# norlab-ulaval/mask_bev

Hardware: AMD Instinct MI355X
Metric: LiDAR scans/sec fwd+bwd, 120k-pt 512x512 BEV 100q (higher is better)
Workload: dtype bf16; 1 GPU; semantic_kitti_512: 120000 pts/scan, 512x512 BEV, 100 queries; scans_per_gpu=4, global_batch=4, parallelism=dp1, step=fwd + Hungarian loss + bwd + AdamW; inputs device-resident, launch=hip-graph, tuned_gemm_table=True, k3_adam_fused=True

## Files before the change

include/maskbev_hip.h:

```cpp
#ifndef MASKBEV_HIP_H_
#define MASKBEV_HIP_H_

#include <stddef.h>
#include <stdint.h>

#ifdef __cplusplus
extern "C" {
#endif

typedef enum {
  MBV_OK = 0,
  MBV_ERR_BAD_ARG = -1,
  MBV_ERR_WORKSPACE = -2,
  MBV_ERR_UNSUPPORTED = -3
} mbv_status;

int mbv_abi_version(void);

#define MBV_DT_F32 0
#define MBV_DT_BF16 1
#define MBV_DT_F16 2

size_t mbv_voxelize_workspace_bytes(int64_t total_points, int32_t batch, int64_t cells_per_scan);

// ... 349 lines not shown
                      int64_t stride_w, int64_t stride_acc, void* stream);

size_t mbv_gemm16_nn_workspace_bytes(int64_t m, int64_t k, int32_t batch);

int mbv_gemm16_nn(const void* g, const void* w, void* out, const void* aux, float* colsum, int64_t m, int64_t n,
                  int64_t k, int64_t ldg, int64_t ldw, int64_t ldo, int64_t ldaux, int32_t dtype, int32_t out_f32,
                  int32_t act, int32_t batch, int64_t stride_g, int64_t stride_w, int64_t stride_o, void* workspace,
                  size_t workspace_bytes, void* stream);

int64_t mbv_gemm16_nn_part_rows(int64_t m, int64_t k, int32_t batch);

int mbv_gemm16_nn_parts(const void* g, const void* w, void* out, const void* aux, float* parts, size_t parts_bytes,
                        int64_t m, int64_t n, int64_t k, int64_t ldg, int64_t ldw, int64_t ldo, int64_t ldaux,
                        int32_t dtype, int32_t out_f32, int32_t act, int32_t batch, int64_t stride_g, int64_t stride_w,
                        int64_t stride_o, void* stream);

size_t mbv_gemm16_tn_workspace_bytes(int64_t m, int64_t n, int64_t k);

int mbv_gemm16_tn(const void* g, const void* x, void* dw, int64_t m, int64_t n, int64_t k, int64_t ldg, int64_t ldx,
                  int64_t lddw, int32_t dtype, int32_t accumulate, int32_t out_f32, int32_t splits, int32_t batch,
                  int64_t stride_g, int64_t stride_x, int64_t stride_dw, void* workspace, size_t workspace_bytes,
                  void* stream);

int mbv_upsample_bilinear_bwd(const void* grad_out, int32_t grad_dtype, int64_t planes, int32_t h, int32_t w, int32_t in_h,
                              int32_t in_w, void* grad_in, int32_t in_dtype, void* stream);

int mbv_groupnorm_supported(int32_t channels, int32_t groups, int32_t h, int32_t w);
size_t mbv_groupnorm_workspace_bytes(int64_t batch, int32_t channels, int32_t groups, int32_t h, int32_t w);
int mbv_groupnorm_fwd(const void* x, int32_t x_dtype, int64_t batch, int32_t channels, int32_t h, int32_t w,
                      int32_t groups, const float* gamma, const float* beta, float eps, const void* add,
// ... 228 lines not shown
```

mask_bev_amd/_lib.py:

```python
from __future__ import annotations

import ctypes
import os
from ctypes import c_double, c_float, c_int32, c_int64, c_size_t, c_void_p
from typing import Dict, List, Tuple

_PKG_DIR = os.path.dirname(os.path.abspath(__file__))
LIB_PATH = os.path.join(_PKG_DIR, 'libmaskbev_hip.so')

ABI_VERSION = 59


class MaskBevHipError(RuntimeError):
    pass


_P = c_void_p
_F = c_float
_I = c_int32
_L = c_int64
_D = c_double

SIGNATURES: Dict[str, Tuple[object, List[object]]] = {
    'mbv_abi_version': (ctypes.c_int, []),
# ... 99 lines not shown
    'mbv_mask_logits_fwd': (ctypes.c_int, [_P, _P, _I, _I, _I, _I, _L, _P, _I, _P]),
    'mbv_attn_mask_from_logits': (ctypes.c_int, [_P, _I, _L, _I, _I, _I, _I, _P, _P]),
    'mbv_attn_workspace_bytes': (c_size_t, [_I, _I, _I, _I, _I]),
    'mbv_attn_fwd': (ctypes.c_int, [_P, _P, _P, _P, _I, _I, _I, _I, _I, _I, _P, _P, _P, c_size_t, _P]),
    'mbv_attn_bwd': (ctypes.c_int, [_P, _P, _P, _P, _P, _P, _P, _I, _I, _I, _I, _I, _I, _P, _P, _P, _P]),
    'mbv_attn_fwd_ld': (ctypes.c_int, [_P, _P, _P, _I, _P, _I, _I, _I, _I, _I, _I, _P, _P, _P, c_size_t, _P]),
    'mbv_gemm16_supported': (ctypes.c_int, [_I, _L, _L, _L]),
    'mbv_gemm16_nt': (ctypes.c_int, [_P, _P, _P, _P, _P, _L, _L, _L, _L, _L, _L, _I, _I, _I, _I, _L, _L, _L, _P]),
    'mbv_gemm16_nt_acc': (ctypes.c_int, [_P, _P, _P, _L, _L, _L, _L, _L, _L, _I, _I, _I, _L, _L, _L, _P]),
    'mbv_gemm16_nn_workspace_bytes': (c_size_t, [_L, _L, _I]),
    'mbv_gemm16_nn': (ctypes.c_int, [_P, _P, _P, _P, _P, _L, _L, _L, _L, _L, _L, _L, _I, _I, _I, _I, _L, _L, _L, _P,
                                     c_size_t, _P]),
    'mbv_gemm16_nn_part_rows': (ctypes.c_int64, [_L, _L, _I]),
    'mbv_gemm16_nn_parts': (ctypes.c_int, [_P, _P, _P, _P, _P, c_size_t, _L, _L, _L, _L, _L, _L, _L, _I, _I, _I, _I, _L,
                                           _L, _L, _P]),
    'mbv_gemm16_tn_workspace_bytes': (c_size_t, [_L, _L, _L]),
    'mbv_gemm16_tn': (ctypes.c_int, [_P, _P, _P, _L, _L, _L, _L, _L, _L, _I, _I, _I, _I, _I, _L, _L, _L, _P, c_size_t,
                                     _P]),
    'mbv_attn_bwd_ld': (ctypes.c_int, [_P, _P, _P, _I, _P, _P, _P, _P, _I, _I, _I, _I, _I, _I, _P, _P, _P, _I, _I, _P]),
    'mbv_msda_query_inputs': (ctypes.c_int, [_P, _P, _L, _L, _I, _I, _P, _P, _P]),
    'mbv_upsample_bilinear_bwd': (ctypes.c_int, [_P, _I, _L, _I, _I, _I, _I, _P, _I, _P]),
    'mbv_groupnorm_supported': (ctypes.c_int, [_I, _I, _I, _I]),
    'mbv_groupnorm_workspace_bytes': (c_size_t, [_L, _I, _I, _I, _I]),
    'mbv_groupnorm_fwd': (ctypes.c_int, [_P, _I, _L, _I, _I, _I, _I, _P, _P, _F, _P, _I, _I, _I, _I, _P, _I, _P, _P, _P,
                                         c_size_t, _P]),
    'mbv_groupnorm_bwd': (ctypes.c_int, [_P, _I, _P, _I, _P, _P, _P, _P, _L, _I, _I, _I, _I, _I, _P, _I, _P, _P, _I, _P,
                                         _P]),
    'mbv_gemm16_tn_group_workspace_bytes': (c_size_t, [_P, _P, _P, _I]),
    'mbv_gemm32s_supported': (ctypes.c_int, [_I, _L, _L, _L]),
    'mbv_f32_absmax_group': (ctypes.c_int, [_P, _P, _P, _P, _P, _I, _P]),
# ... 126 lines not shown
```

mask_bev_amd/csrc/gemm.hip:

```cpp

#include "common.hpp"
#include "gemm_tiles.hpp"

namespace {

template <int KB, int NS, int WM = 2, int TM = 2, int TN = 2>
struct Geo {
  static constexpr int NW = 2 * WM;
  static constexpr int BM = 32 * TM * WM, BN = 64 * TN;
  static constexpr int SA = (BM + 127) / 128, SB = (BN + 127) / 128;
  static constexpr int IMG = 128 * KB * 2;
  static constexpr int STAGE = (SA + SB) * IMG;
  static constexpr int PPS = IMG / 1024;
  static constexpr int PIECES = (SA + SB) * PPS;
  static constexpr int NP = (PIECES + NW - 1) / NW;
  static constexpr int STG = NW * 32 * STG_LD * 4;
  static constexpr int LDS = NS * STAGE > STG ? NS * STAGE : STG;
  static constexpr int BLOCKS = LDS <= 40960 ? 4 : (LDS <= 53248 ? 3 : (LDS <= 81920 ? 2 : 1));
  static constexpr int WPS = (BLOCKS * NW + 3) / 4 > 8 ? 8 : (BLOCKS * NW + 3) / 4;
};

enum { EPI_NONE = 0, EPI_RELU = 1, EPI_GELU = 2, EPI_DRELU = 3, EPI_DGELU = 4,
       EPI_CONV = 5 };

// ... 3 lines not shown
  void* c;
  void* c2;
  const void* aux;
  const float* bias;
  float* colsum_rows;
  int gm, gn, gk;
  int lda, ldb, ldc, ldx;
  long long sa, sb, sc;
  long long ssplit;
  unsigned a_bytes, b_bytes;
  int ntm, ntn, splits, ksteps;
  int out_f32;
  int acc_out;
  int tap_steps;
  int tap[9];
};

template <int KB, int NS, int WM, int TM, int TN, bool A_KS, bool B_KS, int OUT, int EPI, typename T>
__device__ __forceinline__ void gemm16_body(const GemmArgs& p, const int bid, char* smem) {
  using G = Geo<KB, NS, WM, TM, TN>;
  static_assert(OUT == 1 || TN == 2, "the STORE epilogue turns 64-column wave tiles");
  constexpr int BM = G::BM, BN = G::BN;
  const int tid = threadIdx.x, lane = tid & 63;
  const int wave = __builtin_amdgcn_readfirstlane(tid >> 6);
  const int wm = wave >> 1, wn = wave & 1;

  const int tiles = p.ntm * p.ntn;
  const int z = bid / tiles, t = bid - z * tiles;
  const int tile_m = t / p.ntn, tile_n = t - tile_m * p.ntn;
  const int bz = z / p.splits, sp = z - bz * p.splits;
// ... 205 lines not shown
      s += __shfl_xor(s, 32, 64);
      csum[e] = s;
    }
    if (prow == 0 && col_ok) {
      float* d = p.colsum_rows + ((size_t)bz * WM * p.ntm + WM * tile_m + wm) * (size_t)p.gn + gn;
      *reinterpret_cast<float4*>(d) = make_float4(csum[0], csum[1], csum[2], csum[3]);
      *reinterpret_cast<float4*>(d + 4) = make_float4(csum[4], csum[5], csum[6], csum[7]);
    }
  }
}

template <int KB, int NS, int WM, int TM, int TN, bool A_KS, bool B_KS, int OUT, int EPI, typename T>
__global__ void __launch_bounds__(64 * 2 * WM, (Geo<KB, NS, WM, TM, TN>::WPS)) k_gemm16(const GemmArgs p) {
  extern __shared__ __attribute__((aligned(16))) char smem[];
  gemm16_body<KB, NS, WM, TM, TN, A_KS, B_KS, OUT, EPI, T>(p, xcd_contiguous(blockIdx.x, gridDim.x), smem);
}

constexpr int kTnGroup = 48;
struct TnEntry {
  const void* g; const void* x; float* out;
  int m, n, k, ldg, ldx, ldo;
  int ntn, splits, ksteps, item_begin;
};
struct TnGroupArgs {
  TnEntry e[kTnGroup];
  int n, total_items;
};

template <int KB, int NS, typename T>
__global__ void __launch_bounds__(256, (Geo<KB, NS, 2, 2, 2>::WPS)) k_gemm16_tn_group(const TnGroupArgs a) {
// ... 177 lines not shown
  int s = splits;
  if (s <= 0) {
    const long long tiles = (long long)a.ntm * a.ntn * batch;
    constexpr int target = 512;
    s = (int)((target + tiles - 1) / tiles);
    if (s > total_steps * KB / 256) s = total_steps * KB / 256;
  }
  if (s < 1) s = 1;
  if (s > total_steps) s = total_steps;
  a.ksteps = (total_steps + s - 1) / s;
  a.splits = (total_steps + a.ksteps - 1) / a.ksteps;
}

static bool fits_2g(long long rows, long long ld) { return rows * ld * 2 < 0x7fff0000LL; }

extern "C" int mbv_gemm16_supported(int32_t layout, int64_t m, int64_t n, int64_t k) {
  if (layout < 0 || layout > 2 || m <= 0 || n <= 0 || k <= 0) return 0;
  if ((n & 7) || (k & 7)) return 0;
  return m * (n > k ? n : k) * 2 < 0x7fff0000LL ? 1 : 0;
}

extern "C" int mbv_gemm16_nt(const void* x, const void* w, const float* bias, void* out, void* out_pre, int64_t m,
                             int64_t n, int64_t k, int64_t ldx, int64_t ldw, int64_t ldo, int32_t dtype,
                             int32_t out_f32, int32_t act, int32_t batch, int64_t stride_x, int64_t stride_w,
                             int64_t stride_o, void* stream) {
  if (m < 0 || n <= 0 || k <= 0 || batch < 0 || !x || !w || !out) return MBV_ERR_BAD_ARG;
  if (dtype < 0 || dtype > 1 || act < 0 || act > 2) return MBV_ERR_BAD_ARG;
  if ((n & 7) || (k & 7) || (ldx & 7) || (ldw & 7) || (ldo & 7) || ldx < k || ldw < k || ldo < n) return MBV_ERR_UNSUPPORTED;
  if ((reinterpret_cast<size_t>(x) | reinterpret_cast<size_t>(w) | reinterpret_cast<size_t>(out) |
       reinterpret_cast<size_t>(out_pre) | reinterpret_cast<size_t>(bias)) & 15)
    return MBV_ERR_UNSUPPORTED;
  if (!fits_2g(m, ldx) || !fits_2g(n, ldw)) return MBV_ERR_UNSUPPORTED;
  if (m == 0 || batch == 0) return MBV_OK;
  const int shape = gemm16_pick_shape(0, m, n, batch);
  const int BM = SHAPE_BM[shape], BN = SHAPE_BN[shape];
  GemmArgs a = {};
  a.a = x; a.b = w; a.c = out; a.c2 = out_pre; a.bias = bias;
  a.gm = (int)m; a.gn = (int)n; a.gk = (int)k;
  a.lda = (int)ldx; a.ldb = (int)ldw; a.ldc = (int)ldo;
  a.sa = stride_x; a.sb = stride_w; a.sc = stride_o;
  a.a_bytes = (unsigned)(((m - 1) * ldx + k) * 2); a.b_bytes = (unsigned)(((n - 1) * ldw + k) * 2);
  a.ntm = (int)((m + BM - 1) / BM); a.ntn = (int)((n + BN - 1) / BN); a.splits = 1; a.ksteps = (int)((k + KB - 1) / KB);
  a.out_f32 = out_f32;
  return gemm16_launch(shape, 0, 0, act, dtype, a, batch, (hipStream_t)stream);
}

extern "C" int mbv_gemm16_nt_acc(const void* x, const void* w, float* acc, int64_t m, int64_t n, int64_t k, int64_t ldx,
                                 int64_t ldw, int64_t ldacc, int32_t dtype, int32_t splits, int32_t batch,
                                 int64_t stride_x, int64_t stride_w, int64_t stride_acc, void* stream) {
  if (m < 0 || n <= 0 || k <= 0 || batch < 0 || !x || !w || !acc) return MBV_ERR_BAD_ARG;
  if (dtype < 0 || dtype > 1) return MBV_ERR_BAD_ARG;
  if ((n & 7) || (k & 7) || (ldx & 7) || (ldw & 7) || ldx < k || ldw < k || ldacc < n) return MBV_ERR_UNSUPPORTED;
  if ((reinterpret_cast<size_t>(x) | reinterpret_cast<size_t>(w) | reinterpret_cast<size_t>(acc)) & 15) return MBV_ERR_UNSUPPORTED;
  if (!fits_2g(m, ldx) || !fits_2g(n, ldw)) return MBV_ERR_UNSUPPORTED;
  if (m == 0 || batch == 0) return MBV_OK;
  const int shape = gemm16_pick_shape(1, m, n, (long long)batch * ((k + 511) / 512));
  const int BM = SHAPE_BM[shape], BN = SHAPE_BN[shape];
  GemmArgs a = {};
  a.a = x; a.b = w; a.c = acc;
// ... 35 lines not shown
}

extern "C" size_t mbv_gemm16_nn_workspace_bytes(int64_t m, int64_t k, int32_t batch) {
  return (size_t)((m + 63) / 64 + 4) * (size_t)k * 4 * (size_t)(batch > 0 ? batch : 1);
}

extern "C" int64_t mbv_gemm16_nn_part_rows(int64_t m, int64_t k, int32_t batch) {
  if (m <= 0 || k <= 0 || batch <= 0) return 0;
  const int BM = SHAPE_BM[gemm16_pick_shape(0, m, k, batch)];
  return (int64_t)(BM / 64) * ((m + BM - 1) / BM) * batch;
}

static int gemm16_nn_impl(const void* g, const void* w, void* out, const void* aux, float* colsum, bool parts_only, int64_t m,
                          int64_t n, int64_t k, int64_t ldg, int64_t ldw, int64_t ldo, int64_t ldaux, int32_t dtype,
                          int32_t out_f32, int32_t act, int32_t batch, int64_t stride_g, int64_t stride_w,
                          int64_t stride_o, void* workspace, size_t workspace_bytes, void* stream) {
  if (m < 0 || n <= 0 || k <= 0 || batch < 0 || !g || !w || !out) return MBV_ERR_BAD_ARG;
  if (dtype < 0 || dtype > 1 || act < 0 || act > 2 || (act && !aux)) return MBV_ERR_BAD_ARG;
  if ((n & 7) || (k & 7) || (ldg & 7) || (ldw & 7) || (ldo & 7) || (ldaux & 7) || ldg < n || ldw < k || ldo < k)
    return MBV_ERR_UNSUPPORTED;
  if ((reinterpret_cast<size_t>(g) | reinterpret_cast<size_t>(w) | reinterpret_cast<size_t>(out) |
       reinterpret_cast<size_t>(aux) | reinterpret_cast<size_t>(workspace)) & 15)
    return MBV_ERR_UNSUPPORTED;
  if (!fits_2g(m, ldg) || !fits_2g(n, ldw)) return MBV_ERR_UNSUPPORTED;
  const bool sums = colsum != nullptr || parts_only;
  if (sums && (!workspace || workspace_bytes < mbv_gemm16_nn_workspace_bytes(m, k, batch))) return MBV_ERR_WORKSPACE;
  if (m == 0 || batch == 0) return MBV_OK;
  const int shape = gemm16_pick_shape(0, m, k, batch);
  const int BM = SHAPE_BM[shape], BN = SHAPE_BN[shape];
  GemmArgs a = {};
  a.a = g; a.b = w; a.c = out; a.aux = aux; a.colsum_rows = sums ? reinterpret_cast<float*>(workspace) : nullptr;
  a.gm = (int)m; a.gn = (int)k; a.gk = (int)n;
  a.lda = (int)ldg; a.ldb = (int)ldw; a.ldc = (int)ldo; a.ldx = (int)ldaux;
  a.sa = stride_g; a.sb = stride_w; a.sc = stride_o;
  a.a_bytes = (unsigned)(((m - 1) * ldg + n) * 2); a.b_bytes = (unsigned)(((n - 1) * ldw + k) * 2);
  a.ntm = (int)((m + BM - 1) / BM); a.ntn = (int)((k + BN - 1) / BN); a.splits = 1; a.ksteps = (int)((n + KB - 1) / KB);
  a.out_f32 = out_f32;
  const int rc = gemm16_launch(shape, 1, 0, act == 0 ? EPI_NONE : (act == 1 ? EPI_DRELU : EPI_DGELU), dtype, a, batch,
                               (hipStream_t)stream);
  if (rc != MBV_OK || !colsum || parts_only) return rc;
  const int rows = (BM / 64) * a.ntm * batch;
  int gy = rows / 16;
  if (gy < 1) gy = 1;
  if (gy > 32) gy = 32;
  hipLaunchKernelGGL(k_sum_rows, dim3((unsigned)((k + 63) / 64), (unsigned)gy), dim3(256), 0, (hipStream_t)stream,
                     reinterpret_cast<const float*>(workspace), rows, (int)k, colsum);
  MBV_CHECK_LAUNCH();
  return MBV_OK;
}

extern "C" int mbv_gemm16_nn(const void* g, const void* w, void* out, const void* aux, float* colsum, int64_t m,
                             int64_t n, int64_t k, int64_t ldg, int64_t ldw, int64_t ldo, int64_t ldaux, int32_t dtype,
                             int32_t out_f32, int32_t act, int32_t batch, int64_t stride_g, int64_t stride_w,
                             int64_t stride_o, void* workspace, size_t workspace_bytes, void* stream) {
  return gemm16_nn_impl(g, w, out, aux, colsum, false, m, n, k, ldg, ldw, ldo, ldaux, dtype, out_f32, act, batch, stride_g,
                        stride_w, stride_o, workspace, workspace_bytes, stream);
}

extern "C" int mbv_gemm16_nn_parts(const void* g, const void* w, void* out, const void* aux, float* parts, size_t parts_bytes,
                                   int64_t m, int64_t n, int64_t k, int64_t ldg, int64_t ldw, int64_t ldo, int64_t ldaux,
                                   int32_t dtype, int32_t out_f32, int32_t act, int32_t batch, int64_t stride_g,
                                   int64_t stride_w, int64_t stride_o, void* stream) {
  if (!parts) return MBV_ERR_BAD_ARG;
  return gemm16_nn_impl(g, w, out, aux, nullptr, true, m, n, k, ldg, ldw, ldo, ldaux, dtype, out_f32, act, batch, stride_g,
                        stride_w, stride_o, parts, parts_bytes, stream);
}

extern "C" size_t mbv_gemm16_tn_workspace_bytes(int64_t m, int64_t n, int64_t k) {
  const long long tiles = ((n + 127) / 128) * ((k + 127) / 128);
  long long s = (512 + tiles - 1) / tiles;
  const long long cap = (m + 255) / 256;
  if (s > cap) s = cap;
  if (s < 1) s = 1;
  return (size_t)(s + 1) * (size_t)n * (size_t)k * 4;
}

extern "C" int mbv_gemm16_tn(const void* g, const void* x, void* dw, int64_t m, int64_t n, int64_t k, int64_t ldg,
                             int64_t ldx, int64_t lddw, int32_t dtype, int32_t accumulate, int32_t out_f32,
                             int32_t splits, int32_t batch, int64_t stride_g, int64_t stride_x, int64_t stride_dw,
                             void* workspace, size_t workspace_bytes, void* stream) {
// ... 129 lines not shown
```

mask_bev_amd/ops_gemm_kernels.py:

```python
from __future__ import annotations

import ctypes
from typing import Optional

import torch

from . import _lib, switches
from ._lib import MaskBevHipError, check
from .ops_records import *


_GEMM16_DT = {torch.bfloat16: 0, torch.float16: 1}
_ACT = {None: 0, 'none': 0, 'relu': 1, 'gelu': 2}


def gemm16_enabled() -> bool:
    return switches.get('gemm16') != '0'


def gemm16_policy() -> str:
    v = switches.get('gemm16')
    return {'1': 'auto', '0': 'none'}.get(v, v)


def _k17_min_tokens(kind: str) -> Optional[int]:
    return {'fused': switches.get('k17_fused_min'), 'wgrad': 4096}.get(kind)


def _k17_wants(kind: str, tokens: int) -> bool:
    pol = gemm16_policy()
    if pol == 'none':
        return False
    if pol == 'all':
        return True
    floor = _k17_min_tokens(kind)
    return floor is not None and tokens >= floor


def _gemm16_ok(*ts: torch.Tensor) -> bool:
    dt = ts[0].dtype
    return (dt in _GEMM16_DT and all(t.is_cuda and t.dtype == dt and t.dim() == 2 and t.stride(1) == 1
                                     and t.stride(0) % 8 == 0 and t.shape[1] % 8 == 0 and t.data_ptr() % 16 == 0
                                     and t.shape[0] * t.stride(0) * 2 < 0x7fff0000 for t in ts))


def gemm16_nt(x: torch.Tensor, w: torch.Tensor, bias: Optional[torch.Tensor] = None, act: Optional[str] = None,
              out_dtype: Optional[torch.dtype] = None, want_pre: bool = False):
    lib = _lib.load()
    if not _gemm16_ok(x, w) or x.shape[1] != w.shape[1]:
        raise MaskBevHipError('gemm16_nt: unsupported operands')
    m, k = x.shape
    n = w.shape[0]
    od = out_dtype or x.dtype
    if od not in (x.dtype, torch.float32):
        raise MaskBevHipError('gemm16_nt: out dtype must be the input dtype or f32')
    out = torch.empty((m, n), dtype=od, device=x.device)
    pre = torch.empty((m, n), dtype=od, device=x.device) if (want_pre and _ACT[act]) else None
    if bias is not None and (bias.dtype != torch.float32 or not bias.is_contiguous() or bias.data_ptr() % 16):
        raise MaskBevHipError('gemm16_nt: bias must be contiguous f32, 16-byte aligned')
    check(lib.mbv_gemm16_nt(_ptr(x), _ptr(w), _ptr(bias), _ptr(out), _ptr(pre), m, n, k, x.stride(0), w.stride(0), n,
                            _GEMM16_DT[x.dtype], int(od == torch.float32), _ACT[act], 1, 0, 0, 0, _stream()),
          'mbv_gemm16_nt')
    return (out, pre) if want_pre else out


def gemm16_nn(g: torch.Tensor, w: torch.Tensor, act: Optional[str] = None, aux: Optional[torch.Tensor] = None,
              colsum: Optional[torch.Tensor] = None, out_dtype: Optional[torch.dtype] = None, colsum_sink=None) -> torch.Tensor:
    lib = _lib.load()
    if not _gemm16_ok(g, w) or g.shape[1] != w.shape[0]:
        raise MaskBevHipError('gemm16_nn: unsupported operands')
    m, n = g.shape
    k = w.shape[1]
    a = _ACT[act]
    if a and (aux is None or not _gemm16_ok(aux) or aux.dtype != g.dtype or tuple(aux.shape) != (m, k)):
        raise MaskBevHipError('gemm16_nn: aux must be a (M, K) tensor of the input dtype')
    od = out_dtype or g.dtype
    out = torch.empty((m, k), dtype=od, device=g.device)
    if colsum is not None and (colsum.dtype != torch.float32 or not colsum.is_contiguous()):
        raise MaskBevHipError('gemm16_nn: colsum must be contiguous f32')
    if colsum is not None and colsum_sink is not None:
        rows = int(lib.mbv_gemm16_nn_part_rows(m, k, 1))
        parts = torch.empty(int(lib.mbv_gemm16_nn_workspace_bytes(m, k, 1)) // 4, dtype=torch.float32, device=g.device)
        check(lib.mbv_gemm16_nn_parts(_ptr(g), _ptr(w), _ptr(out), _ptr(aux if a else None), _ptr(parts), parts.numel() * 4,
# ... 225 lines not shown
```

mask_bev_amd/switches.py:

```python
from __future__ import annotations

import contextlib
import os
from typing import Any, Dict

_DEFAULTS: Dict[str, Any] = {
    'decoder_fused': 'auto',
    'deferred_heads': True,
    'shared_kv': True,
    'early_targets': True,
    'wgrad_group': True,
    'tn_group': '1',
    'nn_colsum_defer': True,
    'gemm16': 'auto',
    'tn_max_in': 1536,
    'k17_fused_min': 4096,
    'gemm32s': True,
    'amax_hints': True,
    'amax_verify': False,
    'ffn32': True,
    'k4_split': True,
    'k6_split': True,
    'msda_packed_f32': True,
    'ln_bound_hints': True,
    'conv3x3_k20': True,
    'tn32_group': True,
    'gemm32s_min': 1024,
    'pfn_stream_stats': True,
    'pfn_one_call': True,
# ... 60 lines not shown
```

scratch/pmc_to_json.py:

```python
import collections
import csv
import json
import re
import sys

FAMILIES = [
    ('k_gemm16<TN>', r'k_gemm16I.*Lb1ELb1ELi0E', [r'k_add_parts']),
    ('k_gemm16_tn_group', r'k_gemm16_tn_group', [r'k_add_parts_group']),
    ('k_gn_fwd', r'k_gn_apply', [r'k_gn_stats']),
    ('k_gn_bwd', r'k_gn_bwd_dx', [r'k_gn_bwd_sums']),
    ('k_gemm16<NN>', r'k_gemm16I.*Lb0ELb1ELi0E', [r'k_sum_rows']),
    ('k_gemm16<NT>', r'k_gemm16I.*Lb0ELb0ELi0ELi[0-4]E', []),
    ('k_gemm16<NT,conv3x3>', r'k_gemm16I.*Lb0ELb0ELi0ELi5E', []),
    ('k_gemm32s<NT>', r'k_gemm32sILb0ELb0ELi[012]ELi0E|k_gemm32s<false, false, [012], 0>', []),
    ('k_gemm32s<NT,patch>', r'k_gemm32sILb0ELb0ELi0ELi1E|k_gemm32s<false, false, 0, 1>', []),
    ('k_gemm32s<NT,conv3x3>', r'k_gemm32sILb0ELb0ELi0ELi4E|k_gemm32s<false, false, 0, 4>', []),
    ('k_conv_pad_rows', r'k_(un)?pad_rows', []),
    ('k_gemm32s<NN>', r'k_gemm32sILb0ELb1ELi0ELi0E|k_gemm32s<false, true, 0, 0>', []),
    ('k_gemm32s<NN,dact>', r'k_gemm32sILb0ELb1ELi[34]ELi0E|k_gemm32s<false, true, [34], 0>', []),
    ('k_gemm32s<NN,patch>', r'k_gemm32sILb0ELb1ELi0ELi2E|k_gemm32s<false, true, 0, 2>', []),
    ('k_gemm32s<TN>', r'k_gemm32sILb1ELb1ELi0ELi0E|k_gemm32s<true, true, 0, 0>', [r'k_add_parts32']),
    ('k_gemm32s<TN,patch>', r'k_gemm32sILb1ELb1ELi0ELi3E|k_gemm32s<true, true, 0, 3>', []),
    ('k_gemm32s_tn_group', r'k_gemm32s_tn_group', []),
    ('k_absmax_group', r'k_absmax_group', []),
    ('k_adamw', r'k_adamw', []),
    ('k_sample_select', r'k_sample_select', []),
    ('k_window_attn_bwd', r'k_window_attn(_split)?_bwd', []),
# ... 91 lines not shown
```

Measured before the change: 180.6 scans/s.

## Add LDS-resident A-panel GEMM kernel for small-M activated NT/NN GEMMs

Adds a k_gemm16_panel kernel that loads a 128-row A panel with its full K extent into LDS once. It then sweeps a range of N tiles, streaming B through a multi-stage ring buffer, and fuses the bias, activation and colsum epilogues. The scheduler picks how many N ranges to split each panel into based on the CU count. The path is used by default for activated GEMMs with M≤4096 and K≤256, and aims to avoid reloading A for every output tile and to improve occupancy on small GEMMs. The cost is a large LDS footprint and a new code path that needs careful vmcnt bookkeeping.

Measured after the change: 180.2 scans/s. Within noise of the previous version (-0.2%).

```diff
diff --git a/include/maskbev_hip.h b/include/maskbev_hip.h
--- a/include/maskbev_hip.h
+++ b/include/maskbev_hip.h
@@ -387,6 +387,17 @@
                         int64_t m, int64_t n, int64_t k, int64_t ldg, int64_t ldw, int64_t ldo, int64_t ldaux,
                         int32_t dtype, int32_t out_f32, int32_t act, int32_t batch, int64_t stride_g, int64_t stride_w,
                         int64_t stride_o, void* stream);
+
+int mbv_gemm16_panel_nt(const void* x, const void* w, const float* bias, void* out, void* out_pre, int64_t m, int64_t n,
+                        int64_t k, int64_t ldx, int64_t ldw, int64_t ldo, int32_t dtype, int32_t out_f32, int32_t act,
+                        int32_t batch, int64_t stride_x, int64_t stride_w, int64_t stride_o, int32_t n_ranges, void* stream);
+
+int mbv_gemm16_panel_nn(const void* g, const void* w, void* out, const void* aux, float* colsum, int64_t m, int64_t n,
+                        int64_t k, int64_t ldg, int64_t ldw, int64_t ldo, int64_t ldaux, int32_t dtype, int32_t out_f32,
+                        int32_t act, int32_t batch, int64_t stride_g, int64_t stride_w, int64_t stride_o, void* workspace,
+                        size_t workspace_bytes, int32_t n_ranges, void* stream);
+
+int mbv_gemm16_panel_mode(int32_t mode);
 
 size_t mbv_gemm16_tn_workspace_bytes(int64_t m, int64_t n, int64_t k);
 
diff --git a/mask_bev_amd/_lib.py b/mask_bev_amd/_lib.py
--- a/mask_bev_amd/_lib.py
+++ b/mask_bev_amd/_lib.py
@@ -137,6 +137,10 @@
     'mbv_gemm16_nn_part_rows': (ctypes.c_int64, [_L, _L, _I]),
     'mbv_gemm16_nn_parts': (ctypes.c_int, [_P, _P, _P, _P, _P, c_size_t, _L, _L, _L, _L, _L, _L, _L, _I, _I, _I, _I, _L,
                                            _L, _L, _P]),
+    'mbv_gemm16_panel_nt': (ctypes.c_int, [_P, _P, _P, _P, _P, _L, _L, _L, _L, _L, _L, _I, _I, _I, _I, _L, _L, _L, _I, _P]),
+    'mbv_gemm16_panel_nn': (ctypes.c_int, [_P, _P, _P, _P, _P, _L, _L, _L, _L, _L, _L, _L, _I, _I, _I, _I, _L, _L, _L, _P,
+                                           c_size_t, _I, _P]),
+    'mbv_gemm16_panel_mode': (ctypes.c_int, [_I]),
     'mbv_gemm16_tn_workspace_bytes': (c_size_t, [_L, _L, _L]),
     'mbv_gemm16_tn': (ctypes.c_int, [_P, _P, _P, _L, _L, _L, _L, _L, _L, _I, _I, _I, _I, _I, _L, _L, _L, _P, c_size_t,
                                      _P]),
diff --git a/mask_bev_amd/csrc/gemm.hip b/mask_bev_amd/csrc/gemm.hip
--- a/mask_bev_amd/csrc/gemm.hip
+++ b/mask_bev_amd/csrc/gemm.hip
@@ -1,3 +1,5 @@
+
+#include <atomic>
 
 #include "common.hpp"
 #include "gemm_tiles.hpp"
@@ -41,6 +43,8 @@
   int acc_out;
   int tap_steps;
   int tap[9];
+  int nranges;
+  int part_rows;
 };
 
 template <int KB, int NS, int WM, int TM, int TN, bool A_KS, bool B_KS, int OUT, int EPI, typename T>
@@ -276,6 +280,227 @@
 __global__ void __launch_bounds__(64 * 2 * WM, (Geo<KB, NS, WM, TM, TN>::WPS)) k_gemm16(const GemmArgs p) {
   extern __shared__ __attribute__((aligned(16))) char smem[];
   gemm16_body<KB, NS, WM, TM, TN, A_KS, B_KS, OUT, EPI, T>(p, xcd_contiguous(blockIdx.x, gridDim.x), smem);
+}
+
+template <int N>
+__device__ __forceinline__ void wait_vm() { asm volatile("s_waitcnt vmcnt(%0)" ::"n"(N) : "memory"); }
+
+template <int BASE>
+__device__ __forceinline__ void wait_vm_plus(int e) {
+  switch (e) {
+    case 2: wait_vm<BASE + 2>(); break;
+    case 4: wait_vm<BASE + 4>(); break;
+    case 6: wait_vm<BASE + 6>(); break;
+    case 8: wait_vm<BASE + 8>(); break;
+    case 10: wait_vm<BASE + 10>(); break;
+    case 12: wait_vm<BASE + 12>(); break;
+    case 14: wait_vm<BASE + 14>(); break;
+    default: wait_vm<BASE>(); break;
+  }
+}
+
+template <int KB, int NS>
+struct PanelGeo {
+  static constexpr int NW = 8, BM = 128, BN = 128;
+  static constexpr int IMG = 128 * KB * 2;
+  static_assert(IMG / 1024 == NW, "one LDS-DMA piece per wave and sub-image");
+  static constexpr int RING = NS * IMG;
+  static constexpr int SROWS = 16;
+  static constexpr int STG = NW * SROWS * STG_LD * 4;
+  static constexpr int MAX_K = 384;
+  static constexpr int lds_bytes(int ksteps) { return RING + STG + ksteps * IMG; }
+};
+
+template <int KB, int NS, bool B_KS, int EPI, typename T>
+__global__ void __launch_bounds__(512, 2) k_gemm16_panel(const GemmArgs p) {
+  using G = PanelGeo<KB, NS>;
+  extern __shared__ __attribute__((aligned(16))) char smem[];
+  const int tid = threadIdx.x, lane = tid & 63;
+  const int wave = __builtin_amdgcn_readfirstlane(tid >> 6);
+  const int wm = wave >> 1, wn = wave & 1;
+  const int bid = xcd_contiguous(blockIdx.x, gridDim.x);
+  const int pm = bid / p.nranges, rg = bid - pm * p.nranges;
+  const int t_begin = (int)((long long)rg * p.ntn / p.nranges), t_end = (int)((long long)(rg + 1) * p.ntn / p.nranges);
+  const int nk = p.ksteps, m0 = pm * G::BM;
+
+  char* ring = smem;
+  float* stg = reinterpret_cast<float*>(smem + G::RING) + wave * (G::SROWS * STG_LD);
+  char* panel = smem + G::RING + G::STG;
+  const i32x4 ra = make_rsrc(p.a, p.a_bytes), rb = make_rsrc(p.b, p.b_bytes);
+  const unsigned ring_addr = lds_addr_of(ring), panel_addr = lds_addr_of(panel);
+
+  for (int kt = 0; kt < nk; ++kt)
+    glds16(ra, panel_addr + kt * G::IMG + wave * 1024,
+           piece_offset<KB, false>(0, wave, m0, p.gm, p.lda * 2, kt * KB, p.gk, lane), 0u);
+
+  int st_t = t_begin, st_k = 0, st_slot = 0;
+  auto stage = [&]() {
+    unsigned v = OOB;
+    if (st_t < t_end) v = piece_offset<KB, B_KS>(0, wave, st_t * G::BN, p.gn, p.ldb * 2, st_k * KB, p.gk, lane);
+    glds16(rb, ring_addr + st_slot * G::IMG + wave * 1024, v, 0u);
+    if (++st_k == nk) { st_k = 0; ++st_t; }
+    if (++st_slot == NS) st_slot = 0;
+  };
+#pragma unroll
+  for (int s = 0; s < NS - 1; ++s) stage();
+
+  const int r = lane & 31, h = lane >> 5;
+  const int prow = lane >> 3, cg = lane & 7;
+  const int mrow0 = m0 + 32 * wm + prow;
+  constexpr bool HAS_AUX = EPI == EPI_DRELU || EPI == EPI_DGELU;
+  int slot = 0;
+  const int loads_epi = (HAS_AUX ? 4 : 0) + (p.bias ? 2 : 0);
+  const int stores_full = 4 * (((EPI == EPI_RELU || EPI == EPI_GELU) && p.c2) ? 2 : 1);
+  int younger = loads_epi;
+  for (int t = t_begin; t < t_end; ++t) {
+    const int gn = t * G::BN + 64 * wn + 8 * cg;
+    const bool col_ok = gn < p.gn;
+    const bool full = m0 + 32 * wm + 32 <= p.gm && t * G::BN + 64 * wn + 64 <= p.gn;
+    uint4 auxv[4];
+    if (HAS_AUX) {
+#pragma unroll
+      for (int q = 0; q < 4; ++q) {
+        const int gm = mrow0 + 8 * q;
+        const size_t off = (gm < p.gm && col_ok) ? (size_t)gm * p.ldx + gn : 0;
+        auxv[q] = *reinterpret_cast<const uint4*>(reinterpret_cast<const unsigned short*>(p.aux) + off);
+      }
+    }
+    float bias8[8], csum[8];
+#pragma unroll
+    for (int e = 0; e < 8; ++e) { bias8[e] = 0.f; csum[e] = 0.f; }
+    if (p.bias) {
+      const float* bp = p.bias + (col_ok ? gn : 0);
+      const float4 b0 = *reinterpret_cast<const float4*>(bp);
+      const float4 b1 = *reinterpret_cast<const float4*>(bp + 4);
+      bias8[0] = b0.x; bias8[1] = b0.y; bias8[2] = b0.z; bias8[3] = b0.w;
+      bias8[4] = b1.x; bias8[5] = b1.y; bias8[6] = b1.z; bias8[7] = b1.w;
+    }
+    f32x16 acc[2];
+#pragma unroll
+    for (int j = 0; j < 2; ++j)
+#pragma unroll
+      for (int e = 0; e < 16; ++e) acc[j][e] = 0.f;
+    for (int kt = 0; kt < nk; ++kt) {
+      if (kt <= NS - 2) wait_vm_plus<NS - 2>(younger);
+      else wait_vm<NS - 2>();
+      __syncthreads();
+      stage();
+      const char* aimg = panel + kt * G::IMG;
+      const char* bimg = ring + slot * G::IMG;
+      uint4 af[KB / 16], bf[KB / 16][2];
+#pragma unroll
+      for (int ks = 0; ks < KB / 16; ++ks) {
+        af[ks] = frag_kc<KB>(aimg, 32 * wm, ks, lane);
+#pragma unroll
+        for (int j = 0; j < 2; ++j)
+          bf[ks][j] = B_KS ? frag_ks(bimg, 64 * wn + 32 * j, ks, lane) : frag_kc<KB>(bimg, 64 * wn + 32 * j, ks, lane);
+      }
+#pragma unroll
+      for (int ks = 0; ks < KB / 16; ++ks)
+#pragma unroll
+        for (int j = 0; j < 2; ++j) acc[j] = Mma<T>::run(bf[ks][j], af[ks], acc[j]);
+      if (++slot == NS) slot = 0;
+    }
+
+    younger = loads_epi + (full ? stores_full : 0);
+
+#pragma unroll
+    for (int hf = 0; hf < 2; ++hf) {
+      if (hf) __syncthreads();
+      if ((r >> 4) == hf) {
+#pragma unroll
+        for (int j = 0; j < 2; ++j)
+#pragma unroll
+          for (int g = 0; g < 4; ++g) {
+            f32x4 v;
+            v[0] = acc[j][4 * g]; v[1] = acc[j][4 * g + 1]; v[2] = acc[j][4 * g + 2]; v[3] = acc[j][4 * g + 3];
+            *reinterpret_cast<f32x4*>(stg + (r & 15) * STG_LD + 32 * j + 8 * g + 4 * h) = v;
+          }
+      }
+      __syncthreads();
+      if (hf == 0) {
+#pragma unroll
+        for (int e = 0; e < 8; ++e) asm volatile("" : "+v"(bias8[e]));
+        if (HAS_AUX) {
+#pragma unroll
+          for (int q = 0; q < 4; ++q) asm volatile("" : "+v"(auxv[q].x), "+v"(auxv[q].y), "+v"(auxv[q].z), "+v"(auxv[q].w));
+        }
+      }
+#pragma unroll
+      for (int ps = 0; ps < 2; ++ps) {
+        const int row = 8 * ps + prow, q = 2 * hf + ps;
+        const int gm = mrow0 + 8 * q;
+        const f32x4 lo = *reinterpret_cast<const f32x4*>(stg + row * STG_LD + 8 * cg);
+        const f32x4 hi = *reinterpret_cast<const f32x4*>(stg + row * STG_LD + 8 * cg + 4);
+        if (gm >= p.gm || !col_ok) continue;
+        float v[8] = {lo[0], lo[1], lo[2], lo[3], hi[0], hi[1], hi[2], hi[3]};
+#pragma unroll
+        for (int e = 0; e < 8; ++e) v[e] += bias8[e];
+        const size_t o = (size_t)gm * p.ldc + gn;
+        if (EPI == EPI_RELU || EPI == EPI_GELU) {
+          if (p.c2) store8<T>(p.c2, o, v, p.out_f32);
+          if (!p.out_f32) round8<T>(v);
+#pragma unroll
+          for (int e = 0; e < 8; ++e) {
+            if (EPI == EPI_RELU) {
+              v[e] = v[e] > 0.f ? v[e] : 0.f;
+            } else {
+              float dens;
+              v[e] *= gelu_cdf_parts(v[e], dens);
+            }
+          }
+        } else if (HAS_AUX) {
+          const unsigned w[4] = {auxv[q].x, auxv[q].y, auxv[q].z, auxv[q].w};
+#pragma unroll
+          for (int e = 0; e < 8; ++e) {
+            const float zz = Mma<T>::to_f((unsigned short)(w[e >> 1] >> (16 * (e & 1))));
+            if (EPI == EPI_DRELU) {
+              v[e] = zz > 0.f ? v[e] : 0.f;
+            } else {
+              float dens;
+              const float cdf = gelu_cdf_parts(zz, dens);
+              v[e] *= cdf + zz * dens;
+            }
+          }
+        }
+        store8<T>(p.c, o, v, p.out_f32);
+        if (p.colsum_rows) {
+          if (!p.out_f32) round8<T>(v);
+#pragma unroll
+          for (int e = 0; e < 8; ++e) csum[e] += v[e];
+        }
+      }
+    }
+    if (p.colsum_rows) {
+#pragma unroll
+      for (int e = 0; e < 8; ++e) {
+        float s = csum[e];
+        s += __shfl_xor(s, 8, 64);
+        s += __shfl_xor(s, 16, 64);
+        s += __shfl_xor(s, 32, 64);
+        csum[e] = s;
+      }
+      if ((wm & 1) && prow == 0) {
+        *reinterpret_cast<f32x4*>(stg + 8 * cg) = f32x4{csum[0], csum[1], csum[2], csum[3]};
+        *reinterpret_cast<f32x4*>(stg + 8 * cg + 4) = f32x4{csum[4], csum[5], csum[6], csum[7]};
+      }
+      __syncthreads();
+      if (!(wm & 1) && prow == 0 && col_ok) {
+        const float* o = stg + 2 * (G::SROWS * STG_LD);
+        const f32x4 o0 = *reinterpret_cast<const f32x4*>(o + 8 * cg), o1 = *reinterpret_cast<const f32x4*>(o + 8 * cg + 4);
+        float* d = p.colsum_rows + (size_t)(2 * pm + (wm >> 1)) * (size_t)p.gn + gn;
+        *reinterpret_cast<float4*>(d) = make_float4(csum[0] + o0[0], csum[1] + o0[1], csum[2] + o0[2], csum[3] + o0[3]);
+        *reinterpret_cast<float4*>(d + 4) = make_float4(csum[4] + o1[0], csum[5] + o1[1], csum[6] + o1[2], csum[7] + o1[3]);
+        if (pm == p.ntm - 1)
+          for (int row = 2 * p.ntm + (wm >> 1); row < p.part_rows; row += 2) {
+            float* z = p.colsum_rows + (size_t)row * (size_t)p.gn + gn;
+            *reinterpret_cast<float4*>(z) = make_float4(0.f, 0.f, 0.f, 0.f);
+            *reinterpret_cast<float4*>(z + 4) = make_float4(0.f, 0.f, 0.f, 0.f);
+          }
+      }
+    }
+  }
+  asm volatile("s_waitcnt vmcnt(0)" ::: "memory");
 }
 
 constexpr int kTnGroup = 48;
@@ -483,23 +708,113 @@
 
 static bool fits_2g(long long rows, long long ld) { return rows * ld * 2 < 0x7fff0000LL; }
 
+using PG = PanelGeo<KB, NS>;
+constexpr int NS_DEEP = 6;
+using PGD = PanelGeo<KB, NS_DEEP>;
+static bool panel_deep(int ksteps) { return PGD::lds_bytes(ksteps) <= 160 * 1024; }
+
+static std::atomic<int> g_panel_mode{1};
+static std::atomic<int> g_cu_count[64];
+
+static int device_cus(int dev) {
+  int n = dev >= 0 && dev < 64 ? g_cu_count[dev].load(std::memory_order_relaxed) : 0;
+  if (n > 0) return n;
+  if (hipDeviceGetAttribute(&n, hipDeviceAttributeMultiprocessorCount, dev) != hipSuccess || n <= 0) n = 256;
+  if (dev >= 0 && dev < 64) g_cu_count[dev].store(n, std::memory_order_relaxed);
+  return n;
+}
+
+template <int NSP, bool BKS, int EPI, typename T>
+static int panel_launch_n(const GemmArgs& a, int dev, hipStream_t st) {
+  using P = PanelGeo<KB, NSP>;
+  static std::atomic<unsigned long long> ready{0};
+  if (dev < 0 || dev >= 64 || !((ready.load(std::memory_order_acquire) >> dev) & 1ull)) {
+    MBV_CHECK_HIP(hipFuncSetAttribute(reinterpret_cast<const void*>(&k_gemm16_panel<KB, NSP, BKS, EPI, T>),
+                                      hipFuncAttributeMaxDynamicSharedMemorySize, 160 * 1024));
+    if (dev >= 0 && dev < 64) ready.fetch_or(1ull << dev, std::memory_order_release);
+  }
+  hipLaunchKernelGGL((k_gemm16_panel<KB, NSP, BKS, EPI, T>), dim3((unsigned)(a.ntm * a.nranges)), dim3(64 * P::NW),
+                     P::lds_bytes(a.ksteps), st, a);
+  MBV_CHECK_LAUNCH();
+  return MBV_OK;
+}
+
+template <bool BKS, int EPI, typename T>
+static int panel_launch_t(const GemmArgs& a, int dev, hipStream_t st) {
+  return panel_deep(a.ksteps) ? panel_launch_n<NS_DEEP, BKS, EPI, T>(a, dev, st) : panel_launch_n<NS, BKS, EPI, T>(a, dev, st);
+}
+
+template <typename T>
+static int panel_launch_d(int layout, int epi, const GemmArgs& a, int dev, hipStream_t st) {
+  if (layout == 0) {
+    if (epi == EPI_RELU) return panel_launch_t<false, EPI_RELU, T>(a, dev, st);
+    if (epi == EPI_GELU) return panel_launch_t<false, EPI_GELU, T>(a, dev, st);
+    return panel_launch_t<false, EPI_NONE, T>(a, dev, st);
+  }
+  if (epi == EPI_DRELU) return panel_launch_t<true, EPI_DRELU, T>(a, dev, st);
+  if (epi == EPI_DGELU) return panel_launch_t<true, EPI_DGELU, T>(a, dev, st);
+  return panel_launch_t<true, EPI_NONE, T>(a, dev, st);
+}
+
+static bool panel_supported(long long m, long long contraction, long long out, int batch) {
+  return batch == 1 && m > 0 && out > 0 && contraction >= 8 && contraction <= PG::MAX_K && (contraction & 7) == 0 &&
+         (m + PG::BM - 1) / PG::BM * ((out + PG::BN - 1) / PG::BN) <= 0x7fffffffLL;
+}
+
+static int panel_ranges(long long panels, int ntn, int cus) {
+  int best = 1;
+  double best_cost = 0.;
+  for (int r = 1; r <= ntn && r <= 32; ++r) {
+    const long long rounds = (panels * r + cus - 1) / cus;
+    const double cost = (double)rounds * ((ntn + r - 1) / r + 0.5);
+    if (r == 1 || cost < best_cost * 0.999) { best = r; best_cost = cost; }
+  }
+  return best;
+}
+
+static int panel_launch(int layout, int epi, int dtype, GemmArgs a, int n_ranges, hipStream_t st) {
+  int dev = 0;
+  MBV_CHECK_HIP(hipGetDevice(&dev));
+  a.ntm = (a.gm + PG::BM - 1) / PG::BM;
+  a.ntn = (a.gn + PG::BN - 1) / PG::BN;
+  a.ksteps = (a.gk + KB - 1) / KB;
+  a.splits = 1;
+  a.nranges = n_ranges > 0 ? n_ranges : panel_ranges(a.ntm, a.ntn, device_cus(dev));
+  if (a.nranges > a.ntn) a.nranges = a.ntn;
+  if ((long long)a.ntm * a.nranges > 0x7fffffffLL) return MBV_ERR_UNSUPPORTED;
+  return dtype == 0 ? panel_launch_d<__bf16>(layout, epi, a, dev, st) : panel_launch_d<_Float16>(layout, epi, a, dev, st);
+}
+
+constexpr long long PANEL_MAX_ROWS = 4096, PANEL_MAX_CONTRACTION = 256;
+static bool panel_routed(long long m, long long contraction, long long out, int act, int batch) {
+  if (!g_panel_mode.load(std::memory_order_relaxed) || act == 0) return false;
+  return m <= PANEL_MAX_ROWS && contraction <= PANEL_MAX_CONTRACTION && panel_supported(m, contraction, out, batch);
+}
+
+extern "C" int mbv_gemm16_panel_mode(int32_t mode) {
+  if (mode < 0 || mode > 1) return MBV_ERR_BAD_ARG;
+  g_panel_mode.store(mode, std::memory_order_relaxed);
+  return MBV_OK;
+}
+
 extern "C" int mbv_gemm16_supported(int32_t layout, int64_t m, int64_t n, int64_t k) {
   if (layout < 0 || layout > 2 || m <= 0 || n <= 0 || k <= 0) return 0;
   if ((n & 7) || (k & 7)) return 0;
   return m * (n > k ? n : k) * 2 < 0x7fff0000LL ? 1 : 0;
 }
 
-extern "C" int mbv_gemm16_nt(const void* x, const void* w, const float* bias, void* out, void* out_pre, int64_t m,
-                             int64_t n, int64_t k, int64_t ldx, int64_t ldw, int64_t ldo, int32_t dtype,
-                             int32_t out_f32, int32_t act, int32_t batch, int64_t stride_x, int64_t stride_w,
-                             int64_t stride_o, void* stream) {
-  if (m < 0 || n <= 0 || k <= 0 || batch < 0 || !x || !w || !out) return MBV_ERR_BAD_ARG;
+static int gemm16_nt_impl(const void* x, const void* w, const float* bias, void* out, void* out_pre, int64_t m,
+                          int64_t n, int64_t k, int64_t ldx, int64_t ldw, int64_t ldo, int32_t dtype,
+                          int32_t out_f32, int32_t act, int32_t batch, int64_t stride_x, int64_t stride_w,
+                          int64_t stride_o, bool force_panel, int32_t n_ranges, void* stream) {
+  if (m < 0 || n <= 0 || k <= 0 || batch < 0 || n_ranges < 0 || !x || !w || !out) return MBV_ERR_BAD_ARG;
   if (dtype < 0 || dtype > 1 || act < 0 || act > 2) return MBV_ERR_BAD_ARG;
   if ((n & 7) || (k & 7) || (ldx & 7) || (ldw & 7) || (ldo & 7) || ldx < k || ldw < k || ldo < n) return MBV_ERR_UNSUPPORTED;
   if ((reinterpret_cast<size_t>(x) | reinterpret_cast<size_t>(w) | reinterpret_cast<size_t>(out) |
        reinterpret_cast<size_t>(out_pre) | reinterpret_cast<size_t>(bias)) & 15)
     return MBV_ERR_UNSUPPORTED;
   if (!fits_2g(m, ldx) || !fits_2g(n, ldw)) return MBV_ERR_UNSUPPORTED;
+  if (force_panel && (batch == 0 || !panel_supported(m > 0 ? m : 1, k, n, batch))) return MBV_ERR_UNSUPPORTED;
   if (m == 0 || batch == 0) return MBV_OK;
   const int shape = gemm16_pick_shape(0, m, n, batch);
   const int BM = SHAPE_BM[shape], BN = SHAPE_BN[shape];
@@ -509,9 +824,26 @@
   a.lda = (int)ldx; a.ldb = (int)ldw; a.ldc = (int)ldo;
   a.sa = stride_x; a.sb = stride_w; a.sc = stride_o;
   a.a_bytes = (unsigned)(((m - 1) * ldx + k) * 2); a.b_bytes = (unsigned)(((n - 1) * ldw + k) * 2);
+  a.out_f32 = out_f32;
+  if (force_panel || panel_routed(m, k, n, act, batch)) return panel_launch(0, act, dtype, a, n_ranges, (hipStream_t)stream);
   a.ntm = (int)((m + BM - 1) / BM); a.ntn = (int)((n + BN - 1) / BN); a.splits = 1; a.ksteps = (int)((k + KB - 1) / KB);
-  a.out_f32 = out_f32;
   return gemm16_launch(shape, 0, 0, act, dtype, a, batch, (hipStream_t)stream);
+}
+
+extern "C" int mbv_gemm16_nt(const void* x, const void* w, const float* bias, void* out, void* out_pre, int64_t m,
+                             int64_t n, int64_t k, int64_t ldx, int64_t ldw, int64_t ldo, int32_t dtype,
+                             int32_t out_f32, int32_t act, int32_t batch, int64_t stride_x, int64_t stride_w,
+                             int64_t stride_o, void* stream) {
+  return gemm16_nt_impl(x, w, bias, out, out_pre, m, n, k, ldx, ldw, ldo, dtype, out_f32, act, batch, stride_x, stride_w,
+                        stride_o, false, 0, stream);
+}
+
+extern "C" int mbv_gemm16_panel_nt(const void* x, const void* w, const float* bias, void* out, void* out_pre, int64_t m,
+                                   int64_t n, int64_t k, int64_t ldx, int64_t ldw, int64_t ldo, int32_t dtype,
+                                   int32_t out_f32, int32_t act, int32_t batch, int64_t stride_x, int64_t stride_w,
+                                   int64_t stride_o, int32_t n_ranges, void* stream) {
+  return gemm16_nt_impl(x, w, bias, out, out_pre, m, n, k, ldx, ldw, ldo, dtype, out_f32, act, batch, stride_x, stride_w,
+                        stride_o, true, n_ranges, stream);
 }
 
 extern "C" int mbv_gemm16_nt_acc(const void* x, const void* w, float* acc, int64_t m, int64_t n, int64_t k, int64_t ldx,
@@ -577,8 +909,9 @@
 static int gemm16_nn_impl(const void* g, const void* w, void* out, const void* aux, float* colsum, bool parts_only, int64_t m,
                           int64_t n, int64_t k, int64_t ldg, int64_t ldw, int64_t ldo, int64_t ldaux, int32_t dtype,
                           int32_t out_f32, int32_t act, int32_t batch, int64_t stride_g, int64_t stride_w,
-                          int64_t stride_o, void* workspace, size_t workspace_bytes, void* stream) {
-  if (m < 0 || n <= 0 || k <= 0 || batch < 0 || !g || !w || !out) return MBV_ERR_BAD_ARG;
+                          int64_t stride_o, void* workspace, size_t workspace_bytes, bool force_panel, int32_t n_ranges,
+                          void* stream) {
+  if (m < 0 || n <= 0 || k <= 0 || batch < 0 || n_ranges < 0 || !g || !w || !out) return MBV_ERR_BAD_ARG;
   if (dtype < 0 || dtype > 1 || act < 0 || act > 2 || (act && !aux)) return MBV_ERR_BAD_ARG;
   if ((n & 7) || (k & 7) || (ldg & 7) || (ldw & 7) || (ldo & 7) || (ldaux & 7) || ldg < n || ldw < k || ldo < k)
     return MBV_ERR_UNSUPPORTED;
@@ -588,6 +921,7 @@
   if (!fits_2g(m, ldg) || !fits_2g(n, ldw)) return MBV_ERR_UNSUPPORTED;
   const bool sums = colsum != nullptr || parts_only;
   if (sums && (!workspace || workspace_bytes < mbv_gemm16_nn_workspace_bytes(m, k, batch))) return MBV_ERR_WORKSPACE;
+  if (force_panel && (batch == 0 || !panel_supported(m > 0 ? m : 1, n, k, batch))) return MBV_ERR_UNSUPPORTED;
   if (m == 0 || batch == 0) return MBV_OK;
   const int shape = gemm16_pick_shape(0, m, k, batch);
   const int BM = SHAPE_BM[shape], BN = SHAPE_BN[shape];
@@ -599,10 +933,13 @@
   a.a_bytes = (unsigned)(((m - 1) * ldg + n) * 2); a.b_bytes = (unsigned)(((n - 1) * ldw + k) * 2);
   a.ntm = (int)((m + BM - 1) / BM); a.ntn = (int)((k + BN - 1) / BN); a.splits = 1; a.ksteps = (int)((n + KB - 1) / KB);
   a.out_f32 = out_f32;
-  const int rc = gemm16_launch(shape, 1, 0, act == 0 ? EPI_NONE : (act == 1 ? EPI_DRELU : EPI_DGELU), dtype, a, batch,
-                               (hipStream_t)stream);
+  const int rows = (BM / 64) * a.ntm * batch;
+  const int epi = act == 0 ? EPI_NONE : (act == 1 ? EPI_DRELU : EPI_DGELU);
+  a.part_rows = rows;
+  const int rc = force_panel || panel_routed(m, n, k, act, batch)
+                     ? panel_launch(1, epi, dtype, a, n_ranges, (hipStream_t)stream)
+                     : gemm16_launch(shape, 1, 0, epi, dtype, a, batch, (hipStream_t)stream);
   if (rc != MBV_OK || !colsum || parts_only) return rc;
-  const int rows = (BM / 64) * a.ntm * batch;
   int gy = rows / 16;
   if (gy < 1) gy = 1;
   if (gy > 32) gy = 32;
@@ -617,7 +954,16 @@
                              int32_t out_f32, int32_t act, int32_t batch, int64_t stride_g, int64_t stride_w,
                              int64_t stride_o, void* workspace, size_t workspace_bytes, void* stream) {
   return gemm16_nn_impl(g, w, out, aux, colsum, false, m, n, k, ldg, ldw, ldo, ldaux, dtype, out_f32, act, batch, stride_g,
-                        stride_w, stride_o, workspace, workspace_bytes, stream);
+                        stride_w, stride_o, workspace, workspace_bytes, false, 0, stream);
+}
+
+extern "C" int mbv_gemm16_panel_nn(const void* g, const void* w, void* out, const void* aux, float* colsum, int64_t m,
+                                   int64_t n, int64_t k, int64_t ldg, int64_t ldw, int64_t ldo, int64_t ldaux,
+                                   int32_t dtype, int32_t out_f32, int32_t act, int32_t batch, int64_t stride_g,
+                                   int64_t stride_w, int64_t stride_o, void* workspace, size_t workspace_bytes,
+                                   int32_t n_ranges, void* stream) {
+  return gemm16_nn_impl(g, w, out, aux, colsum, false, m, n, k, ldg, ldw, ldo, ldaux, dtype, out_f32, act, batch, stride_g,
+                        stride_w, stride_o, workspace, workspace_bytes, true, n_ranges, stream);
 }
 
 extern "C" int mbv_gemm16_nn_parts(const void* g, const void* w, void* out, const void* aux, float* parts, size_t parts_bytes,
@@ -626,7 +972,7 @@
                                    int64_t stride_w, int64_t stride_o, void* stream) {
   if (!parts) return MBV_ERR_BAD_ARG;
   return gemm16_nn_impl(g, w, out, aux, nullptr, true, m, n, k, ldg, ldw, ldo, ldaux, dtype, out_f32, act, batch, stride_g,
-                        stride_w, stride_o, parts, parts_bytes, stream);
+                        stride_w, stride_o, parts, parts_bytes, false, 0, stream);
 }
 
 extern "C" size_t mbv_gemm16_tn_workspace_bytes(int64_t m, int64_t n, int64_t k) {
diff --git a/mask_bev_amd/ops_gemm_kernels.py b/mask_bev_amd/ops_gemm_kernels.py
--- a/mask_bev_amd/ops_gemm_kernels.py
+++ b/mask_bev_amd/ops_gemm_kernels.py
@@ -37,6 +37,16 @@
     return floor is not None and tokens >= floor
 
 
+_panel_mode_set = [1]
+
+
+def _panel_sync(lib) -> None:
+    mode = 0 if switches.get('gemm16_panel') == '0' else 1
+    if mode != _panel_mode_set[0]:
+        check(lib.mbv_gemm16_panel_mode(mode), 'mbv_gemm16_panel_mode')
+        _panel_mode_set[0] = mode
+
+
 def _gemm16_ok(*ts: torch.Tensor) -> bool:
     dt = ts[0].dtype
     return (dt in _GEMM16_DT and all(t.is_cuda and t.dtype == dt and t.dim() == 2 and t.stride(1) == 1
@@ -47,6 +57,7 @@
 def gemm16_nt(x: torch.Tensor, w: torch.Tensor, bias: Optional[torch.Tensor] = None, act: Optional[str] = None,
               out_dtype: Optional[torch.dtype] = None, want_pre: bool = False):
     lib = _lib.load()
+    _panel_sync(lib)
     if not _gemm16_ok(x, w) or x.shape[1] != w.shape[1]:
         raise MaskBevHipError('gemm16_nt: unsupported operands')
     m, k = x.shape
@@ -67,6 +78,7 @@
 def gemm16_nn(g: torch.Tensor, w: torch.Tensor, act: Optional[str] = None, aux: Optional[torch.Tensor] = None,
               colsum: Optional[torch.Tensor] = None, out_dtype: Optional[torch.dtype] = None, colsum_sink=None) -> torch.Tensor:
     lib = _lib.load()
+    _panel_sync(lib)
     if not _gemm16_ok(g, w) or g.shape[1] != w.shape[0]:
         raise MaskBevHipError('gemm16_nn: unsupported operands')
     m, n = g.shape
diff --git a/mask_bev_amd/switches.py b/mask_bev_amd/switches.py
--- a/mask_bev_amd/switches.py
+++ b/mask_bev_amd/switches.py
@@ -13,6 +13,7 @@
     'tn_group': '1',
     'nn_colsum_defer': True,
     'gemm16': 'auto',
+    'gemm16_panel': 'auto',
     'tn_max_in': 1536,
     'k17_fused_min': 4096,
     'gemm32s': True,
diff --git a/scratch/pmc_to_json.py b/scratch/pmc_to_json.py
--- a/scratch/pmc_to_json.py
+++ b/scratch/pmc_to_json.py
@@ -9,8 +9,8 @@
     ('k_gemm16_tn_group', r'k_gemm16_tn_group', [r'k_add_parts_group']),
     ('k_gn_fwd', r'k_gn_apply', [r'k_gn_stats']),
     ('k_gn_bwd', r'k_gn_bwd_dx', [r'k_gn_bwd_sums']),
-    ('k_gemm16<NN>', r'k_gemm16I.*Lb0ELb1ELi0E', [r'k_sum_rows']),
-    ('k_gemm16<NT>', r'k_gemm16I.*Lb0ELb0ELi0ELi[0-4]E', []),
+    ('k_gemm16<NN>', r'k_gemm16I.*Lb0ELb1ELi0E|k_gemm16_panelILi\d+ELi\d+ELb1E', [r'k_sum_rows']),
+    ('k_gemm16<NT>', r'k_gemm16I.*Lb0ELb0ELi0ELi[0-4]E|k_gemm16_panelILi\d+ELi\d+ELb0E', []),
     ('k_gemm16<NT,conv3x3>', r'k_gemm16I.*Lb0ELb0ELi0ELi5E', []),
     ('k_gemm32s<NT>', r'k_gemm32sILb0ELb0ELi[012]ELi0E|k_gemm32s<false, false, [012], 0>', []),
     ('k_gemm32s<NT,patch>', r'k_gemm32sILb0ELb0ELi0ELi1E|k_gemm32s<false, false, 0, 1>', []),
diff --git a/scratch/ubench/k17_panel_measure.py b/scratch/ubench/k17_panel_measure.py
--- /dev/null
+++ b/scratch/ubench/k17_panel_measure.py
@@ -0,0 +1,131 @@
+import json
+import math
+import os
+import sys
+
+import torch
+
+sys.path.insert(0, os.path.dirname(os.path.dirname(os.path.dirname(os.path.abspath(__file__)))))
+from mask_bev_amd import _lib
+
+lib = _lib.load()
+dev = torch.device('cuda', 0)
+dt = torch.bfloat16
+SETS = 3
+
+
+def p(t):
+    return None if t is None else t.data_ptr()
+
+
+def stream():
+    return torch.cuda.current_stream().cuda_stream
+
+
+def timeit_batch(fn, n=40, reps=7):
+    for i in range(6):
+        fn(i % SETS)
+    torch.cuda.synchronize()
+    ts = []
+    for _ in range(reps):
+        a, b = torch.cuda.Event(enable_timing=True), torch.cuda.Event(enable_timing=True)
+        a.record()
+        for i in range(n):
+            fn(i % SETS)
+        b.record()
+        b.synchronize()
+        ts.append(a.elapsed_time(b) * 1e3 / n)
+    ts.sort()
+    return ts[len(ts) // 2], ts[0]
+
+
+def nt_case(m, c, o, act, want_pre):
+    xs = [torch.randn(m, c, device=dev).to(dt) for _ in range(SETS)]
+    w = (torch.randn(o, c, device=dev) / math.sqrt(c)).to(dt)
+    b = torch.randn(o, device=dev)
+    outs = [torch.empty(m, o, device=dev, dtype=dt) for _ in range(SETS)]
+    pres = [torch.empty(m, o, device=dev, dtype=dt) if want_pre else None for _ in range(SETS)]
+
+    def tile(i):
+        rc = lib.mbv_gemm16_nt(p(xs[i]), p(w), p(b), p(outs[i]), p(pres[i]), m, o, c, c, c, o, 0, 0, act, 1, 0, 0, 0, stream())
+        assert rc == 0, rc
+
+    def panel(nr):
+        def f(i):
+            rc = lib.mbv_gemm16_panel_nt(p(xs[i]), p(w), p(b), p(outs[i]), p(pres[i]), m, o, c, c, c, o, 0, 0, act, 1, 0, 0, 0, nr,
+                                         stream())
+            assert rc == 0, rc
+        return f
+    return tile, panel
+
+
+def nn_case(m, c, o, act, sums):
+    gs = [torch.randn(m, c, device=dev).to(dt) for _ in range(SETS)]
+    w = (torch.randn(c, o, device=dev) / math.sqrt(c)).to(dt)
+    auxs = [torch.randn(m, o, device=dev).to(dt) for _ in range(SETS)]
+    outs = [torch.empty(m, o, device=dev, dtype=dt) for _ in range(SETS)]
+    nbytes = int(lib.mbv_gemm16_nn_workspace_bytes(m, o, 1))
+    parts = torch.empty(nbytes // 4, device=dev) if sums else None
+
+    def tile(i):
+        if sums:
+            rc = lib.mbv_gemm16_nn_parts(p(gs[i]), p(w), p(outs[i]), p(auxs[i]), p(parts), nbytes, m, c, o, c, o, o, o, 0, 0, act, 1, 0,
+                                         0, 0, stream())
+        else:
+            rc = lib.mbv_gemm16_nn(p(gs[i]), p(w), p(outs[i]), p(auxs[i]), None, m, c, o, c, o, o, o, 0, 0, act, 1, 0, 0, 0, None, 0,
+                                   stream())
+        assert rc == 0, rc
+
+    def panel(nr):
+        def f(i):
+            if sums and m <= 4096:
+                lib.mbv_gemm16_panel_mode(1)
+                rc = lib.mbv_gemm16_nn_parts(p(gs[i]), p(w), p(outs[i]), p(auxs[i]), p(parts), nbytes, m, c, o, c, o, o, o, 0, 0, act,
+                                             1, 0, 0, 0, stream())
+                lib.mbv_gemm16_panel_mode(0)
+            else:
+                rc = lib.mbv_gemm16_panel_nn(p(gs[i]), p(w), p(outs[i]), p(auxs[i]), None, m, c, o, c, o, o, o, 0, 0, act, 1, 0, 0, 0, None,
+                                             0, nr, stream())
+            assert rc == 0, rc
+        return f
+    return tile, panel
+
+
+CASES = [
+    ('swin1 fc1+gelu', 'nt', 65536, 192, 768, 2, True),
+    ('swin1 fc2 dgrad*gelu\'', 'nn', 65536, 192, 768, 2, True),
+    ('swin2 fc1+gelu', 'nt', 16384, 384, 1536, 2, True),
+    ('swin2 fc2 dgrad*gelu\'', 'nn', 16384, 384, 1536, 2, True),
+    ('pixdec fc1+relu', 'nt', 21504, 256, 1024, 1, False),
+    ('pixdec fc2 dgrad*relu\'', 'nn', 21504, 256, 1024, 1, True),
+    ('8192 fc1+gelu', 'nt', 8192, 192, 768, 2, True),
+    ('8192 fc2 dgrad*gelu\'', 'nn', 8192, 192, 768, 2, True),
+    ('4096 fc1+gelu', 'nt', 4096, 192, 768, 2, True),
+    ('4096 fc2 dgrad*gelu\'', 'nn', 4096, 192, 768, 2, True),
+    ('4096 c384 fc1+gelu', 'nt', 4096, 384, 1536, 2, True),
+    ('4096 c256 fc1+relu', 'nt', 4096, 256, 1024, 1, False),
+    ('4096 c256 fc2 dgrad*relu\'', 'nn', 4096, 256, 1024, 1, True),
+    ('2048 fc1+gelu', 'nt', 2048, 192, 768, 2, True),
+    ('2048 fc2 dgrad*gelu\'', 'nn', 2048, 192, 768, 2, True),
+    ('1024 fc1+gelu', 'nt', 1024, 192, 768, 2, True),
+    ('512 c256 fc1+relu', 'nt', 512, 256, 2048, 1, False),
+]
+
+res = []
+for name, kind, m, c, o, act, flag in CASES:
+    tile, panel = (nt_case(m, c, o, act, flag) if kind == 'nt' else nn_case(m, c, o, act, flag))
+    lib.mbv_gemm16_panel_mode(0)
+    t_med, t_min = timeit_batch(tile)
+    p_med, p_min = timeit_batch(panel(0))
+    t2_med, t2_min = timeit_batch(tile)
+    p2_med, p2_min = timeit_batch(panel(0))
+    row = dict(name=name, m=m, c=c, o=o, tile_us=[round(t_med, 1), round(t2_med, 1)], panel_us=[round(p_med, 1), round(p2_med, 1)],
+               gain_pct=round(100 * (1 - min(p_med, p2_med) / min(t_med, t2_med)), 1),
+               gain_worst_pct=round(100 * (1 - max(p_med, p2_med) / min(t_med, t2_med)), 1))
+    print(json.dumps(row), flush=True)
+    res.append(row)
+    del tile, panel
+    torch.cuda.empty_cache()
+lib.mbv_gemm16_panel_mode(1)
+with open(sys.argv[1] if len(sys.argv) > 1 else 'k17_panel_measure.json', 'w') as fh:
+    json.dump(res, fh, indent=1)
```
